# t-neumann/versalignLib

Hardware: AMD Instinct MI355X
Metric: GCUPS (giga DP cell updates/sec) SW affine-gap, 150x500 bp (higher is better)
Workload: dtype int16; 1 GPU; 1048576 pairs/GPU, 150 bp x 500 bp, SW affine-gap int16 score (open -5, extend -1), inputs resident in HBM; pairs_per_gpu=1048576, read_length=150, ref_length=500, kernel_geometry=8x19

## Files before the change

versalignlib_amd/csrc/cell_constants.h:

```cpp
#pragma once

namespace valign {

struct Scoring {
    int match = 2, mismatch = -1, gap_read = -3, gap_ref = -3;
    bool affine = false;
    int open_read = -3, ext_read = -3, open_ref = -3, ext_ref = -3;
};

constexpr int kAlgSW = 0;
constexpr int kAlgNW = 1;

constexpr int kGapLinear = 0, kGapSym = 1, kGapAffine = 2, kGapAffineSym = 3;
constexpr int kGapAffineSymF16 = 4, kGapAffineF16 = 5, kGapSymF16 = 6;
constexpr int kTiltMaxK = 12;
constexpr int kSideTileG = 8, kSideTileK = 19;
constexpr bool tilt_tables_only(int G, int K) { return G == kSideTileG && K == kSideTileK; }
constexpr bool tilt_frame_built(int G, int K) { return K <= kTiltMaxK || tilt_tables_only(G, K); }
constexpr int kSideTilePad = kSideTileG + 4, kSideTilePairs = 2 * (64 / kSideTileG);
constexpr int side_tile_refs_area(int F) { return ((kSideTilePairs * F + 32 + 15) / 16) * 16; }
constexpr int side_tile_stream_stride(int F) {
    const int dw = (F + 2 * kSideTilePad + 1) / 2;
    return 4 * (dw + ((kSideTileG - dw) % 64 + 64) % 64);
}
constexpr int side_tile_wave_lds(int R, int F) {
    const int streams = (64 / kSideTileG) * side_tile_stream_stride(F), raw_reads = ((kSideTilePairs * R + 32 + 15) / 16) * 16;
    return side_tile_refs_area(F) + (streams > raw_reads ? streams : raw_reads);
}

constexpr int kBandNwAbsent16 = -16384;
constexpr int kBandNwAbsent32 = -(1 << 29);

enum FillKernel {
    kFillLinear = 0,
    kFillLinearSym,
    kFillAffine,
    kFillSse,
    kFillTag,
    kFillTagKey,
    kFillAffineSym,
    kFillAffineTag,
    kFillAffineTagSym,
    kFillSseTag,
// ... 7 lines not shown
```

versalignlib_amd/csrc/cell_rules.h:

```cpp
#pragma once

#include <algorithm>
#include <cstdlib>
#include <stdexcept>
#include <string>

#include "cell_constants.h"
#include "extend_band_align_plan.h"

namespace valign {

struct RuleInputs {
    Scoring sc;
    int R = 0, F = 0;
    bool sse_policy = false;
    bool no_sym = false, no_tag = false, no_f16 = false, no_prof_key = false;
    bool no_max3 = false;
    bool no_tilt = false;
    bool no_row_tables = false;
    bool no_side_tile = false;
};

inline long long nw_tilt_span(const Scoring &sc, int rows, int F) {
    const long long per_row = -(long long)(sc.affine ? sc.ext_ref : sc.gap_ref);
    const long long per_col = -(long long)(sc.affine ? sc.ext_read : sc.gap_read);
    return per_row * (rows + 1) + per_col * (F + 1);
}

inline bool half_float_exact(const Scoring &sc, int alg, int R, int F, int rows) {
    const long long top = (long long)std::min(R, F) * std::max({sc.match, sc.mismatch, 0});
    long long slack = std::max({std::abs(sc.match), std::abs(sc.mismatch), std::abs(sc.open_read),
                                std::abs(sc.ext_read), std::abs(sc.open_ref), std::abs(sc.ext_ref)});
    if (alg == kAlgSW) return top + 2 * slack <= 2048 && slack <= 1024;
    if (!sc.affine) slack = std::max<long long>(slack, std::max(std::abs(sc.gap_read), std::abs(sc.gap_ref)));
    const long long span = nw_tilt_span(sc, rows, F);
// ... 123 lines not shown
    return std::max({sc.match, sc.mismatch, 0}) - 2 * sc.ext_ref + (sc.ext_ref - sc.open_ref);
}
inline bool sym_affine_row_tables_ok(const RuleInputs &in, int R, int F, int rows, int K, int lds_profile, int lds_tables) {
    if (in.no_row_tables || !sym_affine_tilt_ok(in, R, F, rows, K)) return false;
    if (in.sc.ext_ref - in.sc.open_ref < 0 || F > 60000) return false;
    return sym_affine_row_table_low(in.sc) >= 0 && sym_affine_row_table_high(in.sc) <= 255 && lds_tables <= lds_profile;
}
inline const char *ran_sym_affine_scores_name(bool row_tables) { return row_tables ? "row_tables" : "lds_profile"; }

constexpr int kSideTileRows = kSideTileG * kSideTileK, kSideTileMinRead = 129;
constexpr int kSideTileBlockWaves = 4, kSideTileLdsGranule = 2048, kSideTileLdsBudget = 152 * 1024;
inline bool side_tile_lds_ok(int lds_wave) {
    const long long block = ((long long)lds_wave * kSideTileBlockWaves + kSideTileLdsGranule - 1) / kSideTileLdsGranule * kSideTileLdsGranule;
    return lds_wave > 0 && 2 * block <= kSideTileLdsBudget;
}
inline const char *sym_affine_side_tile_refusal(const RuleInputs &in, int alg, int gaps, int R, int F, bool latency, bool forced) {
    const int lds_wave = side_tile_wave_lds(R, F);
    if (in.no_side_tile) return "the side tile is switched off (VALIGN_HIP_DEBUG=no_side_tile)";
    if (alg != kAlgSW) return "the 8 x 19 tile exists for Smith-Waterman scores only";
    if (gaps != kGapAffineSym)
        return "the 8 x 19 tile exists for int16 cells with symmetric affine gaps only (half_float_cells = 0, open_read = open_ref, ext_read = ext_ref)";
    if (R > kSideTileRows) return "the 8 x 19 tile holds reads of at most 152 bases";
    if (in.no_tilt) return "the 8 x 19 tile runs the tilted frame only (VALIGN_HIP_DEBUG=no_tilt)";
    if (in.no_row_tables) return "the 8 x 19 tile runs the row tables only (VALIGN_HIP_DEBUG=no_row_tables)";
    if (!sym_affine_row_tables_ok(in, in.R, in.F, kSideTileRows, kSideTileK, lds_wave, lds_wave))
        return "the 8 x 19 tile runs the tilted frame with row tables only: shape x scoring leave its window, or a substitution score of the frame is no byte (sym_affine_row_tables_ok)";
    if (!side_tile_lds_ok(lds_wave)) return "the 8 x 19 tile needs two 4-wave blocks per CU: the reference is too long for its LDS budget";
    if (forced) return "";
    if (R < kSideTileMinRead) return "reads of at most 128 bases fit a smaller tile";
    if (latency) return "small calls take the latency plan";
// ... 395 lines not shown
```

versalignlib_amd/csrc/dp_kernels.hip.h:

```cpp
#pragma once

#include <hip/hip_runtime.h>
#include <stdint.h>

#include <type_traits>
#include <utility>

#include "base_classes.h"
#include "cell_constants.h"
#include "lane_map.h"

namespace valign {

typedef short s16x2 __attribute__((ext_vector_type(2)));
typedef _Float16 f16x2 __attribute__((ext_vector_type(2)));
typedef unsigned short u16x2 __attribute__((ext_vector_type(2)));

constexpr int kWave = 64;
constexpr int kWaveLanes = 64;
constexpr int kCodePad = 72;
constexpr short kNegInf = -16384;

constexpr int kMaxScoreGroups = 16;
constexpr int kOneSweep = 0x7FFFFFFF;
// ... 396 lines not shown
    w.refc = refc + 2 * kCodePad;
    w.first_bad = first_bad;
    w.pair0 = pair0;
    w.last = last;
    return live;
}

constexpr int row_table_pad(int G) { return G + 4; }
constexpr unsigned kSelZero4 = 0x0c0c0c0cu;
constexpr unsigned kSelWiden = 0x04010400u;

template <int G, int K>
__device__ __forceinline__ bool wave_setup_tables(const uint8_t *reads, const uint8_t *refs, long long n, int R, int F,
                                                  int refs_area, int sel_stride, int wave_lds, short match, short mismatch,
                                                  short zero_score, short row0_score, unsigned block, WaveTables &w,
                                                  unsigned (&Ta)[K], unsigned (&Tb)[K], bool &repair) {
    using geo = Geo<G, K>;
    constexpr int kPad = row_table_pad(G);
    const int lane = threadIdx.x & (kWave - 1);
    const int wave = threadIdx.x / kWave;
    const int row0 = R - geo::kRows;

    unsigned char *raw = valign_smem + (size_t)wave * wave_lds;
    unsigned char *sel = raw + refs_area;

    const int waves = blockDim.x / kWave;
    const long long pair0 = ((long long)block * waves + wave) * geo::kPairs;
    const bool live = pair0 < n;
    long long pair_end = pair0 + geo::kPairs;
    if (pair_end > n) pair_end = n;
    const int last = (int)(pair_end - pair0) - 1;

    if (live) {
        stage_span(raw, refs, pair0 * F, pair_end * F, lane);
        stage_span(sel, reads, pair0 * R, pair_end * R, lane);
    }
    __syncthreads();

    if (live) {
        auto table = [&](int c, unsigned &lo, unsigned &hi) __attribute__((always_inline)) {
            unsigned b[8];
#pragma unroll
            for (int a = 0; a < 8; ++a) b[a] = (unsigned)(a >= 1 && a <= 4 ? (a == c + 1 ? match : mismatch) : zero_score) & 0xFFu;
            lo = b[0] | b[1] << 8 | b[2] << 16 | b[3] << 24;
            hi = b[4] | b[5] << 8 | b[6] << 16 | b[7] << 24;
        };
        unsigned t_lo[4], t_hi[4];
#pragma unroll
        for (int c = 0; c < 4; ++c) table(c, t_lo[c], t_hi[c]);
// ... 35 lines not shown
#pragma unroll
        for (int q = 0; q < K; ++q) {
            Ta[q] += r4;
            Tb[q] += r4;
        }
    }
    __syncthreads();

    int cols_used = 0;
    bool before_last = false;
    unsigned *stream = reinterpret_cast<unsigned *>(sel);
    const int stride_dw = sel_stride / 4;
    constexpr bool SEL16 = tilt_tables_only(G, K);
    unsigned short *stream16 = reinterpret_cast<unsigned short *>(sel);
    const int stride_h = sel_stride / 2;
    if (live) {
        for (int idx = lane; idx < geo::kGroups * 2 * kPad; idx += kWave) {
            const int g = idx / (2 * kPad), x = idx - g * (2 * kPad);
            if constexpr (SEL16) stream16[g * stride_h + (x < kPad ? x : F + x)] = (unsigned short)0x0c0c;
            else stream[g * stride_dw + (x < kPad ? x : F + x)] = kSelZero4;
        }
        const int ref_skew = (int)((unsigned long long)(refs + pair0 * F) & 15ull);
        typedef unsigned short u16;
#pragma unroll
        for (int g = 0; g < geo::kGroups; ++g) {
            int pa = 2 * g, pb = 2 * g + 1;
            pa = pa > last ? last : pa;
            pb = pb > last ? last : pb;
            const unsigned char *raw_a = raw + ref_skew + pa * F, *raw_b = raw + ref_skew + pb * F;
            unsigned *out_g = stream + g * stride_dw + kPad;
            unsigned short *out16_g = stream16 + g * stride_h + kPad;
            u16x2 ends_a = u16x2{0, 0}, ends_b = u16x2{0, 0};
            auto note = [](u16x2 &ends, unsigned acgt, int j) __attribute__((always_inline)) {
                const unsigned none = ~nonzero_bytes(acgt) & 0x80808080u;
                const u16 end = acgt ? (u16)(j + 4 - (__builtin_clz(acgt) >> 3)) : (u16)0;
                const u16 first_none = none ? (u16)(0xFFFF - (j + (__builtin_ctz(none) >> 3))) : (u16)0;
                ends = __builtin_elementwise_max(ends, u16x2{end, first_none});
            };
            const int F4 = F & ~3;
            for (int j = 4 * lane; j < F4; j += 4 * kWave) {
                const unsigned ca = base_class4(lds_dword_at(raw_a + j)), cb = base_class4(lds_dword_at(raw_b + j));
                const unsigned sa = select_bytes8(0x0c0c0c03u, 0x0201000cu, ca), sb = select_bytes8(0x0c0c0c07u, 0x0605040cu, cb);
                if constexpr (SEL16) {
                    uint2 s;
                    s.x = __builtin_amdgcn_perm(sb, sa, 0x05010400u);
                    s.y = __builtin_amdgcn_perm(sb, sa, 0x07030602u);
                    *reinterpret_cast<uint2 *>(out16_g + j) = s;
                } else {
                    uint4 s;
                    s.x = __builtin_amdgcn_perm(sb, sa, 0x0c040c00u) | 0x0c000c00u;
                    s.y = __builtin_amdgcn_perm(sb, sa, 0x0c050c01u) | 0x0c000c00u;
                    s.z = __builtin_amdgcn_perm(sb, sa, 0x0c060c02u) | 0x0c000c00u;
                    s.w = __builtin_amdgcn_perm(sb, sa, 0x0c070c03u) | 0x0c000c00u;
                    *reinterpret_cast<uint4 *>(out_g + j) = s;
                }
                note(ends_a, sa ^ kSelZero4, j);
                note(ends_b, sb ^ kSelZero4, j);
            }
            for (int j = F4 + lane; j < F; j += kWave) {
                const int ca = base_class(raw_a[j]), cb = base_class(raw_b[j]);
                const bool va = ca >= 1 && ca <= 4, vb = cb >= 1 && cb <= 4;
                if constexpr (SEL16) out16_g[j] = (unsigned short)((va ? (unsigned)(ca - 1) : 0x0cu) | (vb ? (unsigned)(cb + 3) : 0x0cu) << 8);
                else out_g[j] = (va ? (unsigned)(ca - 1) : 0x0cu) | (vb ? (unsigned)(cb + 3) : 0x0cu) << 16 | 0x0c000c00u;
                ends_a = __builtin_elementwise_max(ends_a, u16x2{va ? (u16)(j + 1) : (u16)0, va ? (u16)0 : (u16)(0xFFFF - j)});
                ends_b = __builtin_elementwise_max(ends_b, u16x2{vb ? (u16)(j + 1) : (u16)0, vb ? (u16)0 : (u16)(0xFFFF - j)});
            }
#pragma unroll
            for (int d = kWave / 2; d >= 1; d >>= 1) {
                ends_a = __builtin_elementwise_max(ends_a, __builtin_bit_cast(u16x2, __shfl_xor(__builtin_bit_cast(int, ends_a), d, kWave)));
                ends_b = __builtin_elementwise_max(ends_b, __builtin_bit_cast(u16x2, __shfl_xor(__builtin_bit_cast(int, ends_b), d, kWave)));
            }
            before_last |= 0xFFFF - (int)ends_a.y < (int)ends_a.x || 0xFFFF - (int)ends_b.y < (int)ends_b.x;
            cols_used = (int)ends_a.x > cols_used ? (int)ends_a.x : cols_used;
            cols_used = (int)ends_b.x > cols_used ? (int)ends_b.x : cols_used;
        }
    }
    __syncthreads();
    repair = __builtin_amdgcn_readfirstlane((int)before_last) != 0;
    w.cols_used = __builtin_amdgcn_readfirstlane(cols_used);
    w.prof = raw;
    w.refc = SEL16 ? reinterpret_cast<unsigned char *>(stream16 + kPad) : reinterpret_cast<unsigned char *>(stream + kPad);
    w.first_bad = nullptr;
    w.pair0 = pair0;
    w.last = last;
    return live;
}

template <int K>
__device__ __forceinline__ void lds_load_lane(unsigned addr, unsigned (&v)[K / 2]) {
// ... 32 lines not shown
    lds_load_lane<K>(addr_b, vb);
    merge_profile<K>(va, vb, S);
}



constexpr int kTrackAll = 0, kTrackNone = 1, kTrackPair = 2;

__host__ __device__ inline int nw_frame_centre(int R, int F, int rows, int match, int mismatch, int tilt_row, int tilt_col) {
    const int best = match > mismatch ? match : mismatch;
    const int top = (R < F ? R : F) * (best > 0 ? best : 0);
    return (top + tilt_row * (rows + 1) + tilt_col * (F + 1)) / 2;
}

template <int G, int K, int ALG, int GAPS>
__global__ void __launch_bounds__(256)
score_kernel(const ScoreArgs args) {
    using geo = Geo<G, K>;
    constexpr bool F16 = GAPS == kGapAffineSymF16 || GAPS == kGapAffineF16;
    constexpr bool F16SYM = GAPS == kGapAffineSymF16;
    constexpr bool AFFINE = GAPS == kGapAffine || GAPS == kGapAffineSym || F16;
    constexpr bool SYM = GAPS == kGapSym;
    constexpr bool LINF16 = GAPS == kGapSymF16;
    constexpr bool AFFSYM = GAPS == kGapAffineSym;
    constexpr bool SOURCES = AFFSYM && ALG == kAlgSW;
    const int lane = threadIdx.x & (kWave - 1);
    using lmap = LaneMap<G, score_lane_stride(G, K)>;
    static_assert(lmap::kInterleaved || (lmap::grp(kWave - 3) == (kWave - 3) / G && lmap::l(kWave - 3) == (kWave - 3) % G), "the contiguous map is lane / G, lane % G");
    const int grp = lmap::kInterleaved ? lmap::grp(lane) : lane / G;
    const int l = lmap::kInterleaved ? lmap::l(lane) : lane % G;

    const uint8_t *reads = args.reads, *refs = args.refs;
    int16_t *scores = args.scores;
    long long n_pairs = args.n;
    int F_batch = args.F;
    unsigned block = blockIdx.x;
    if (args.n_groups > 0) {
        int g = 0;
        while (g + 1 < args.n_groups && block >= args.groups[g].block_end) ++g;
        block -= g ? args.groups[g - 1].block_end : 0u;
        reads += args.groups[g].read_ofs;
        refs += args.groups[g].ref_ofs;
        scores += args.groups[g].pair_ofs;
        n_pairs = args.groups[g].n;
        F_batch = args.groups[g].F;
// ... 23 lines not shown
    auto cell_add = [](s16x2 a, s16x2 b) __attribute__((always_inline)) {
        return HALF ? __builtin_bit_cast(s16x2, __builtin_bit_cast(f16x2, a) + __builtin_bit_cast(f16x2, b)) : a + b;
    };
    auto cell_sub = [](s16x2 a, s16x2 b) __attribute__((always_inline)) {
        return HALF ? __builtin_bit_cast(s16x2, __builtin_bit_cast(f16x2, a) - __builtin_bit_cast(f16x2, b)) : a - b;
    };
    const short s_match = HALF ? __builtin_bit_cast(short, (_Float16)(((int)args.match + fold) * unit)) : (short)(args.match + fold);
    const short s_mismatch = HALF ? __builtin_bit_cast(short, (_Float16)(((int)args.mismatch + fold) * unit)) : (short)(args.mismatch + fold);
    const short s_zero = HALF ? __builtin_bit_cast(short, (_Float16)fold) : (short)fold;
    bool tables = false, repair = false;
    unsigned Ta[K], Tb[K];
    if constexpr (TABLES_ONLY) {
        tables = args.sym_max3_bias > 0 && (args.sym_max3_bias >> 16 & 3) == 3;
        if (!tables) return;
        if (!wave_setup_tables<G, K>(reads, refs, n_pairs, args.R, F_batch, args.prof_area, args.refc_stride, args.wave_lds,
                                     s_match, s_mismatch, s_zero, s_row0, block, w, Ta, Tb, repair))
            return;
        if (args.form_seen != nullptr && lane == 0) args.form_seen[repair ? 1 : 0] = 1u;
    } else if constexpr (TILT_BUILT) {
        tables = args.sym_max3_bias > 0 && (args.sym_max3_bias >> 16 & 3) == 3;
        bool live = false;
        if (tables)
            live = wave_setup_tables<G, K>(reads, refs, n_pairs, args.R, F_batch, args.prof_area, args.refc_stride, args.wave_lds,
                                           s_match, s_mismatch, s_zero, s_row0, block, w, Ta, Tb, repair);
        if (!tables)
            live = wave_setup<G, K, false>(reads, refs, n_pairs, args.R, F_batch, args.prof_area, args.refc_stride,
                                           args.wave_lds, s_match, s_mismatch, w, false, block, s_zero, kOneSweep, 0, s_row0);
        if (!live) return;
    } else if (!wave_setup<G, K, false>(reads, refs, n_pairs, args.R, F_batch, args.prof_area, args.refc_stride,
                                        args.wave_lds, s_match, s_mismatch, w, false, block, s_zero, kOneSweep, 0, s_row0))
        return;
// ... 506 lines not shown
            res = s16x2{(short)((int)b.x + rcentre), (short)((int)b.y + rcentre)};
        } else {
            res = s16x2{(short)(int)b.x, (short)(int)b.y};
        }
    } else if (ALG == kAlgSW) {
        res = best;
    } else {
        s16x2 col = l == G - 1 ? row_best : pk(0);
#pragma unroll
        for (int q = 0; q < K; ++q) col = pk_max(col, Hl[q] - cell(tilt_row * (l * K + q) + tilt_col * F));
        res = pk_max(col, pk(0));
    }
#pragma unroll
    for (int i = 0; i < lmap::kReduceSteps; ++i)
        res = pk_max(res, as_pk((unsigned)__shfl_xor((int)as_u32(res), lmap::reduce_distance(i), kWave)));
    if (l == 0) {
        const long long pa = pair0 + 2 * grp;
        if (pa + 1 < n_pairs && ((unsigned long long)scores & 3ull) == 0) {
            *reinterpret_cast<unsigned *>(scores + pa) = as_u32(res);
        } else {
            if (pa < n_pairs) scores[pa] = res.x;
            if (pa + 1 < n_pairs) scores[pa + 1] = res.y;
        }
    }
}

struct WaveLds {
    int prof_area, refc_stride, total;
};

template <int G, int K>
inline WaveLds wave_lds(int R, int F) {
// ... 33 lines not shown
```

versalignlib_amd/csrc/engine.hip.h:

```cpp
#pragma once

#include <hip/hip_runtime.h>
#include <stdint.h>
#include <stdio.h>
#include <stdlib.h>
#include <string.h>

#include <algorithm>
#include <atomic>
#include <chrono>
#include <condition_variable>
#include <functional>
#include <map>
#include <memory>
#include <mutex>
#include <stdexcept>
#include <string>
#include <thread>
#include <utility>
#include <vector>

#include "align_parts.h"
#include "cell_rules.h"
#include "hip_handles.h"
// ... 98 lines not shown
#undef VALIGN_COUNT

extern const Geometry kSideGeometry;

constexpr int kMaxBlockLds = 160 * 1024;
static_assert(kSideTileLdsBudget < kMaxBlockLds, "the side tile's LDS budget leaves a margin inside a CU's LDS");
constexpr int kSlots = 4;
constexpr int kDefaultBlockLds = 64 * 1024;

struct LaunchPlan {
    bool long_mode = false;
    const Geometry *geo = nullptr;
    WaveLds lds{};
    int waves_per_block = 4;
    int pairs_per_wave = 0;
};

class DebugSwitches {
public:
    DebugSwitches() {
        const char *env = getenv("VALIGN_HIP_DEBUG");
        if (!env) return;
        static const char *const known[] = {"no_sym", "no_tag", "no_f16", "no_max3", "no_tilt", "no_row_tables", "no_side_tile", "no_fused", "no_prof_key", "no_overlap", "no_band_chain",
                                            "force_long", "wide_align", "strip_k", "no_single_strip", "no_direct_out", "ragged_min", "chunk_bytes",
                                            "align_chunk_bytes", "direct_bytes", "scratch_cap_mb", "whole_rows", "short_strips", "cigar_rows_mb", "cigar_lanes",
                                            "span_scratch_bytes", "subopt_scratch_bytes", "span_cigar_mb"};
        std::string s(env);
        for (size_t at = 0; at <= s.size();) {
            const size_t end = std::min(s.find(',', at), s.size());
            const std::string item = s.substr(at, end - at);
            at = end + 1;
            if (item.empty()) continue;
            const size_t eq = item.find('=');
            const std::string name = item.substr(0, eq);
            bool ok = false;
            for (const char *k : known) ok = ok || name == k;
            if (!ok) throw std::runtime_error("VALIGN_HIP_DEBUG: unknown switch '" + name + "'");
            kv_[name] = eq == std::string::npos ? 1 : atoll(item.c_str() + eq + 1);
// ... 134 lines not shown
    void score_long_device(int alg, long long n, const uint8_t *d_reads, const uint8_t *d_refs, int16_t *d_scores, hipStream_t stream);
    void sync_band_tables(hipStream_t stream);
    void score_band_device(const LongScoreMode &mode, long long n, const uint8_t *d_reads, const uint8_t *d_refs, int16_t *d_scores, PlacedRec *d_placed,
                           hipStream_t stream);

    const char *score_cell_format(int alg, long long n = 0) const;
    std::string ran_score_cells() const;
    const char *ran_align_fill() const { return ran_align_fill_; }
    static std::string ran_geometry(const Geometry *g) { return g ? std::to_string(g->G) + "x" + std::to_string(g->K) : "none"; }
    std::string ran_kernels() const;

    RuleInputs rule_inputs() const {
        RuleInputs in = RuleInputs{sc_, R_, F_, sse_policy_, no_sym_, no_tag_, no_f16_, no_prof_key_, no_max3_, no_tilt_};
        in.no_row_tables = no_row_tables_;
        in.no_side_tile = no_side_tile_;
        return in;
    }
    bool score_int16_ok(int alg) const;
    bool score_wide_cells(int alg) const { return score_width_ == 32 || (score_width_ == 0 && !score_int16_ok(alg)); }

    void score_host(int opt, int n, const char *const *reads, const char *const *refs, short *scores,
                    int threads, int16_t *d_dest = nullptr);



    struct WalkChain {
        int region;
        long long chunk_pairs;
        int *min_start;
        uint8_t *packed;
// ... 138 lines not shown
    PlacedSweep extend_wide_sweep(ExtendRec *d_extend, bool banded = false) const;
    PlacedSweep extend_band_sweep() const;
    void score_placed_strips(const PlacedSweep &sweep, long long n, const uint8_t *d_reads, const uint8_t *d_refs, hipStream_t stream);
    static void raise_block_lds(const void *fn, int bytes) {
        if (bytes > kDefaultBlockLds)
            hip_check(hipFuncSetAttribute(fn, hipFuncAttributeMaxDynamicSharedMemorySize, bytes), "hipFuncSetAttribute(MaxDynamicSharedMemorySize)");
    }
    TraceArgs trace_args(int alg, const uint8_t *d_reads, const uint8_t *d_refs, long long n, const unsigned *ptr, const EndCell *ends, uint8_t *rows,
                         short *idx, int G, int K, int pad_rows, int blocks8) const;

    LaunchPlan choose_plan(int R, int F, int force_g, int force_k, bool latency = false, bool full_only = false) const;

    static LaunchPlan long_plan();

    LaunchPlan score_plan_for(const LaunchPlan &base, int alg, int R, int F, bool latency, bool refuse = true) const;
    static LaunchPlan side_plan(int R, int F);
    const char *side_tile_refusal(int alg, int R, int F, bool latency) const;
    bool few_pairs(long long n) const { return n > 0 && n <= (long long)latency_plan_.pairs_per_wave * 1024 && band_width_ == 0; }
    const char *ran_side_tile_form() const;
    void reset_side_tile_form(hipStream_t stream);


    long long whole_rounds(long long pairs, bool sw_scores = false) const;

    bool direct_call(long long n, size_t per_pair) const;

    void prime_copy_engines(hipStream_t copy_in, hipStream_t copy_out, long long staged_pairs);

    void flat_destination(FlatSink sink, long long n, uint8_t *&rows, short *&idx) const {
        if (HostRegistry::instance().covers(sink.rows, (size_t)n * 2 * sink.AL) &&
            HostRegistry::instance().covers(sink.idx, sizeof(short) * 4 * (size_t)n)) {
// ... 239 lines not shown
    std::vector<int> read_caps_, ref_caps_;
    std::vector<unsigned char> read_class_;
    std::vector<unsigned short> ref_class_;
    std::map<std::pair<int, int>, LaunchPlan> class_plans_;
    hipStream_t ragged_dev_stream_ = nullptr;
    HostPacker packer_{R_, F_};
    HostStats host_stats_;
    DebugSwitches dbg_;
    bool no_sym_ = dbg_.on("no_sym");
    bool no_tag_ = dbg_.on("no_tag");
    bool no_f16_ = dbg_.on("no_f16");
    bool no_max3_ = dbg_.on("no_max3");
    bool no_tilt_ = dbg_.on("no_tilt");
    bool no_row_tables_ = dbg_.on("no_row_tables");
    bool no_side_tile_ = dbg_.on("no_side_tile");
    bool side_forced_ = false;
    bool no_fused_ = dbg_.on("no_fused");
    bool no_prof_key_ = dbg_.on("no_prof_key");
    bool copy_engines_primed_ = false;
    std::unique_ptr<CopyIssuer> copy_issuer_;
    bool wide_align_ = dbg_.on("wide_align");
    bool whole_rows_ = dbg_.on("whole_rows");
    bool no_direct_out_ = dbg_.on("no_direct_out");
    bool no_overlap_ = dbg_.on("no_overlap");
    int strip_k_ = (int)dbg_.value("strip_k", 0);
    long long scratch_cap_mb_ = dbg_.value("scratch_cap_mb", 0);
    bool chain_regions_busy_[2] = {false, false};
    std::string arch_;
    LaunchPlan plan_, latency_plan_;
    LaunchPlan base_plan_;
// ... 3 lines not shown
    long long staged_pairs_ = 0, align_staged_pairs_ = 0;
    size_t record_staged_bytes_ = 0;
    bool pack_ = true;
    BandPlan band_plan_;
    int band_tables_width_ = -1;
    int band_blocks_per_cu_ = 0, band_lds_ = 0;
    int long_strip_rows_ = 0;
    static constexpr unsigned kRanF16 = 1, kRanInt16 = 2, kRanInt32 = 4;
    unsigned ran_score_cells_ = 0;
    const char *ran_align_fill_ = "none";
    const Geometry *ran_score_geo_ = nullptr, *ran_align_geo_ = nullptr;
    const Geometry *ran_placed_geo_ = nullptr, *ran_subopt_geo_ = nullptr, *ran_extend_geo_ = nullptr;
    const char *ran_score_sym_affine_ = nullptr;
    const char *ran_score_sym_affine_frame_ = "plain";
    const char *ran_score_sym_affine_scores_ = "lds_profile";
    const char *ran_placed_ = "none";
    std::string ran_span_ = "none";
    size_t span_scratch_bytes_ = (size_t)dbg_.value("span_scratch_bytes", 256ll << 20);
    std::string ran_span_cigar_ = "none";
    size_t span_cigar_bytes_ = (size_t)std::max(0ll, dbg_.value("span_cigar_mb", 768)) << 20;
    const char *ran_subopt_ = "none";
    int subopt_ring_cols_ = 0;
    size_t subopt_scratch_bytes_ = (size_t)dbg_.value("subopt_scratch_bytes", 256ll << 20);
    const char *ran_extend_ = "none";
    const char *ran_extend_align_ = "none";
    const Geometry *ran_extend_align_geo_ = nullptr;
    long long ran_extend_align_chunks_ = 0;
    const char *ran_result_format_ = "rows";
    int ran_cigar_lanes_ = 0;
    long long cigar_d2h_bytes_ = 0;
// ... 54 lines not shown
```

versalignlib_amd/csrc/engine_core.hip:

```cpp
#include <numeric>

#include "engine.hip.h"

namespace valign {

static WaveLds side_tile_lds(int R, int F) { return row_table_lds16(R, F); }
static Geometry side_geometry() {
    Geometry g{kSideTileG, kSideTileK, false, &side_tile_lds, {}, {}, [](int, int) -> const void * { return nullptr; },
               [](int, int) -> const void * { return nullptr; }, [](int) -> const void * { return nullptr; }, [](int) -> const void * { return nullptr; }};
    g.kernel[kAlgSW][kGapAffineSym] = (const void *)&score_kernel<kSideTileG, kSideTileK, kAlgSW, kGapAffineSym>;
    return g;
}
const Geometry kSideGeometry = side_geometry();

Engine::Engine(int device, int R, int F, const Scoring &sc, int force_g, int force_k)
    : device_(device), R_(R), F_(F), sc_(sc) {
    if (R < 0 || F < 0) throw std::runtime_error("negative sequence length");
    if ((long long)R + F > 32767)
        throw std::runtime_error("read_length + ref_length exceeds the ABI's 16-bit coordinates");
    validate_scoring();
    int count = 0;
    hip_check(hipGetDeviceCount(&count), "hipGetDeviceCount");
    if (device < 0 || device >= count)
        throw std::runtime_error("HIP device " + std::to_string(device) + " not present (" +
// ... 109 lines not shown
             (long long)(d_cig_rows_[0].bytes() + d_cig_rows_[1].bytes()), ran_placed_, placed_wide(), (long long)(d_placed_rows_.bytes() + d_placed_ends_.bytes()),
             ran_span_.c_str(), span_ref_length(rule_inputs()), (long long)span_[kSlots].bytes(),
             ran_span_cigar_.c_str(), (long long)(span_cigar_[0].bytes() + span_cigar_[1].bytes()),
             ran_subopt_, (long long)subopt_[kSlots].bytes(), subopt_ring_cols_, ran_extend_, extend_wide(), extend_band(), VALIGN_HIP_EXTEND_BAND_BLOCK_ROWS,
             ran_geometry(ran_score_geo_).c_str(), ran_geometry(ran_align_geo_).c_str(),
             ran_geometry(ran_placed_geo_).c_str(), ran_geometry(ran_subopt_geo_).c_str(), ran_geometry(ran_extend_geo_).c_str());
    std::string out(buf);
    out.insert(out.size() - 1, std::string(", \"ran_extend_align\": \"") + ran_extend_align_ + "\", \"ran_extend_align_geometry\": \"" +
                                   ran_geometry(ran_extend_align_geo_) + "\", \"extend_align_scratch_bytes\": " +
                                   std::to_string((long long)(d_ptr_.bytes() + d_ends_.bytes() + d_extend_align_recs_.bytes())) +
                                   ", \"extend_band_align\": " + std::to_string(extend_band_align()) + ", \"ran_extend_align_chunks\": " +
                                   std::to_string(ran_extend_align_chunks_) + ", \"ran_cigar_lanes\": " + std::to_string(ran_cigar_lanes_));
    if (ran_score_sym_affine_)
        out.insert(out.size() - 1, std::string(", \"ran_score_sym_affine\": \"") + ran_score_sym_affine_ + "\", \"ran_score_sym_affine_frame\": \"" +
                                       ran_score_sym_affine_frame_ + "\", \"ran_score_sym_affine_scores\": \"" + ran_score_sym_affine_scores_ + "\"");
    if (ran_score_sym_affine_ && ran_score_geo_ == &kSideGeometry)
        out.insert(out.size() - 1, std::string(", \"ran_score_sym_affine_form\": \"") + ran_side_tile_form() + "\"");
    return out;
}

void Engine::band_block_shape(int &block_rows, int &col_align) const {
    const bool chain = long_mode(kAlgSW, false).chain;
    block_rows = chain ? kBandK : VALIGN_HIP_BAND_BLOCK_ROWS;
    col_align = chain ? VALIGN_HIP_BAND_CHAIN_COL_ALIGN : VALIGN_HIP_BAND_COL_ALIGN;
}

void Engine::validate_scoring() {
    auto fits = [](int v) { return v >= -32768 && v <= 32767; };
    if (!fits(sc_.match) || !fits(sc_.mismatch) || !fits(sc_.gap_read) || !fits(sc_.gap_ref) ||
        !fits(sc_.open_read) || !fits(sc_.ext_read) || !fits(sc_.open_ref) || !fits(sc_.ext_ref))
        throw std::runtime_error("scoring parameter outside int16");
    const bool gaps_ok = sc_.affine ? (sc_.open_read <= 0 && sc_.ext_read <= 0 && sc_.open_ref <= 0 && sc_.ext_ref <= 0)
// ... 39 lines not shown
        if (latency) cost = (double)(F + g.G - 1) * (g.K * (sc_.affine ? 9.3 : 5.6) + 7.0);
        if (!best.geo || cost < best_cost) {
            best = p;
            best_cost = cost;
        }
    }
    if (!best.geo || (dbg_.on("force_long") && !force_g)) {
        if (force_g || force_k)
            throw std::runtime_error("the forced kernel geometry does not fit read_length=" + std::to_string(R) +
                                     ", ref_length=" + std::to_string(F));
        return long_plan();
    }
    return best;
}

LaunchPlan Engine::side_plan(int R, int F) {
    LaunchPlan p;
    p.geo = &kSideGeometry;
    p.lds = kSideGeometry.lds(R, F);
    p.waves_per_block = kSideTileBlockWaves;
    p.pairs_per_wave = 2 * (kWave / kSideTileG);
    return p;
}

const char *Engine::side_tile_refusal(int alg, int R, int F, bool latency) const {
    const RuleInputs in = rule_inputs();
    const int gaps = alg <= kAlgNW ? score_gap_form(in, alg, R, F, kSideTileRows) : -1;
    return sym_affine_side_tile_refusal(in, alg, gaps, R, F, latency, side_forced_);
}

const char *Engine::ran_side_tile_form() const {
    if (!d_form_seen_.get()) return "none";
    unsigned seen[2] = {0, 0};
    hip_check(hipSetDevice(device_), "hipSetDevice");
// ... 146 lines not shown
```

versalignlib_amd/csrc/engine_score.hip:

```cpp
#define VALIGN_TU_SCORE 1
#include "engine.hip.h"

namespace valign {

void Engine::score_device(int opt, long long n, const uint8_t *d_reads, const uint8_t *d_refs,
                  int16_t *d_scores, hipStream_t stream, bool length_sorted) {
    const int alg = opt & 0xF;
    if (alg > 1 || n <= 0) return;
    hip_check(hipSetDevice(device_), "hipSetDevice");
    if (length_sorted) {
        host_stats_ = HostStats{};
        ran_score_cells_ = 0;
        ran_score_geo_ = nullptr;
        ran_score_sym_affine_ = nullptr;
        reset_side_tile_form(stream);
    }
    if (score_width_ == 16 && !score_int16_ok(alg))
        throw std::runtime_error("shape x scoring can leave the int16 range of the DP cells (read_length " +
                                 std::to_string(R_) + ", ref_length " + std::to_string(F_) + ")");
    const bool wide = score_wide_cells(alg);
    if (side_forced_ && (plan_.long_mode || wide || band_width_ > 0))
        throw std::runtime_error("group_lanes = 8, rows_per_lane = 19: the call takes the long-read kernels (a band, int32 cells, or a reference too long for the register sweep)");
    if (plan_.long_mode || wide) {
        score_long_device(alg, n, d_reads, d_refs, d_scores, stream);
// ... 52 lines not shown
    ran_score_geo_ = plan.geo;
    if (alg == kAlgSW && gaps == kGapAffineSym) {
        const bool max3 = sym_affine_max3_ok(rule_inputs(), R_, F_);
        a.sym_max3_bias = max3 ? sym_affine_bias(sc_) : 0;
        const bool tilted = sym_affine_tilt_ok(rule_inputs(), R_, F_, plan.geo->G * plan.geo->K, plan.geo->K);
        if (tilted) a.sym_max3_bias = sym_affine_tilt_bias(sc_) | 1 << 16;
        const WaveLds tables_lds = tilt_tables_only(plan.geo->G, plan.geo->K) ? plan.lds : row_table_lds(plan.geo->G, R, F);
        const bool row_tables = tilted && sym_affine_row_tables_ok(rule_inputs(), R_, F_, plan.geo->G * plan.geo->K, plan.geo->K, plan.lds.total, tables_lds.total);
        if (tilt_tables_only(plan.geo->G, plan.geo->K)) {
            if (!row_tables) throw std::runtime_error("the 8 x 19 side tile was planned for a launch whose row tables are refused");
            if (!d_form_seen_.get()) {
                d_form_seen_.reserve(2 * sizeof(unsigned), "side tile form words");
                hip_check(hipMemset(d_form_seen_.get(), 0, 2 * sizeof(unsigned)), "hipMemset(form words)");
            }
            a.form_seen = d_form_seen_.get();
        }
        if (row_tables) {
            a.sym_max3_bias |= 1 << 17;
            a.prof_area = tables_lds.prof_area;
            a.refc_stride = tables_lds.refc_stride;
            a.wave_lds = tables_lds.total;
        }
        ran_score_sym_affine_ = ran_sym_affine_name(max3);
        ran_score_sym_affine_frame_ = ran_sym_affine_frame_name(tilted);
        ran_score_sym_affine_scores_ = ran_sym_affine_scores_name(row_tables);
    }
    const int block_lds = a.wave_lds * plan.waves_per_block;
    if (block_lds > kDefaultBlockLds)
        hip_check(hipFuncSetAttribute(fn, hipFuncAttributeMaxDynamicSharedMemorySize, block_lds),
                  "hipFuncSetAttribute(MaxDynamicSharedMemorySize)");
    if (blocks > 0x7FFFFFFFll) throw std::runtime_error("batch too large for one launch");
    if (blocks == 0) return;
    void *kargs[] = {&a};
    hip_check(hipLaunchKernel(fn, dim3((unsigned)blocks), dim3(plan.waves_per_block * kWave), kargs,
                              (size_t)block_lds, stream),
              "hipLaunchKernel(score_kernel)");
}

void Engine::launch_unpack(const uint8_t *d_packed, uint8_t *d_out, long long n, int len, hipStream_t stream) {
    if (n <= 0 || len <= 0) return;
    UnpackArgs a{d_packed, d_out, n, len};
    void *kargs[] = {&a};
// ... 358 lines not shown
```

Before: 10690 GCUPS.

## Stage side-tile references in halves to fit three blocks per CU

```diff
diff --git a/versalignlib_amd/csrc/cell_constants.h b/versalignlib_amd/csrc/cell_constants.h
--- a/versalignlib_amd/csrc/cell_constants.h
+++ b/versalignlib_amd/csrc/cell_constants.h
@@ -27,6 +27,10 @@
     const int streams = (64 / kSideTileG) * side_tile_stream_stride(F), raw_reads = ((kSideTilePairs * R + 32 + 15) / 16) * 16;
     return side_tile_refs_area(F) + (streams > raw_reads ? streams : raw_reads);
 }
+constexpr int side_tile_refs_half_area(int F) { return ((kSideTilePairs / 2 * F + 32 + 15) / 16) * 16; }
+constexpr int side_tile_half_staged_wave_lds(int R, int F) {
+    return side_tile_wave_lds(R, F) - side_tile_refs_area(F) + side_tile_refs_half_area(F);
+}
 
 constexpr int kBandNwAbsent16 = -16384;
 constexpr int kBandNwAbsent32 = -(1 << 29);
diff --git a/versalignlib_amd/csrc/cell_rules.h b/versalignlib_amd/csrc/cell_rules.h
--- a/versalignlib_amd/csrc/cell_rules.h
+++ b/versalignlib_amd/csrc/cell_rules.h
@@ -19,6 +19,7 @@
     bool no_tilt = false;
     bool no_row_tables = false;
     bool no_side_tile = false;
+    bool no_side_tile_3 = false;
 };
 
 inline long long nw_tilt_span(const Scoring &sc, int rows, int F) {
@@ -172,6 +173,25 @@
     const long long block = ((long long)lds_wave * kSideTileBlockWaves + kSideTileLdsGranule - 1) / kSideTileLdsGranule * kSideTileLdsGranule;
     return lds_wave > 0 && 2 * block <= kSideTileLdsBudget;
 }
+constexpr int kSideTileTwoBlockLds = 56 * 1024;
+inline bool side_tile_lds_ok3(int lds_wave) {
+    const long long block = ((long long)lds_wave * kSideTileBlockWaves + kSideTileLdsGranule - 1) / kSideTileLdsGranule * kSideTileLdsGranule;
+    return lds_wave > 0 && 3 * block <= kSideTileLdsBudget;
+}
+struct SideTileLayout {
+    int blocks_per_cu;
+    bool half_staged;
+    int refs_area;
+    int wave_lds;
+    int block_lds;
+};
+inline SideTileLayout side_tile_layout(const RuleInputs &in, int R, int F) {
+    const int half = side_tile_half_staged_wave_lds(R, F), full = side_tile_wave_lds(R, F);
+    if (!in.no_side_tile_3 && side_tile_lds_ok3(half))
+        return SideTileLayout{3, true, side_tile_refs_half_area(F), half, half * kSideTileBlockWaves};
+    return SideTileLayout{2, false, side_tile_refs_area(F), full, std::max(full * kSideTileBlockWaves, kSideTileTwoBlockLds)};
+}
+
 inline const char *sym_affine_side_tile_refusal(const RuleInputs &in, int alg, int gaps, int R, int F, bool latency, bool forced) {
     const int lds_wave = side_tile_wave_lds(R, F);
     if (in.no_side_tile) return "the side tile is switched off (VALIGN_HIP_DEBUG=no_side_tile)";
diff --git a/versalignlib_amd/csrc/dp_kernels.hip.h b/versalignlib_amd/csrc/dp_kernels.hip.h
--- a/versalignlib_amd/csrc/dp_kernels.hip.h
+++ b/versalignlib_amd/csrc/dp_kernels.hip.h
@@ -434,9 +434,10 @@
 __device__ __forceinline__ bool wave_setup_tables(const uint8_t *reads, const uint8_t *refs, long long n, int R, int F,
                                                   int refs_area, int sel_stride, int wave_lds, short match, short mismatch,
                                                   short zero_score, short row0_score, unsigned block, WaveTables &w,
-                                                  unsigned (&Ta)[K], unsigned (&Tb)[K], bool &repair) {
+                                                  unsigned (&Ta)[K], unsigned (&Tb)[K], bool &repair, bool half_staged = false) {
     using geo = Geo<G, K>;
     constexpr int kPad = row_table_pad(G);
+    constexpr int kHalfPairs = geo::kPairs / 2, kHalfGroups = geo::kGroups / 2;
     const int lane = threadIdx.x & (kWave - 1);
     const int wave = threadIdx.x / kWave;
     const int row0 = R - geo::kRows;
@@ -451,8 +452,9 @@
     if (pair_end > n) pair_end = n;
     const int last = (int)(pair_end - pair0) - 1;
 
+    const bool second_half = half_staged && last >= kHalfPairs;
     if (live) {
-        stage_span(raw, refs, pair0 * F, pair_end * F, lane);
+        stage_span(raw, refs, pair0 * F, (second_half ? pair0 + kHalfPairs : pair_end) * F, lane);
         stage_span(sel, reads, pair0 * R, pair_end * R, lane);
     }
     __syncthreads();
@@ -518,65 +520,147 @@
     constexpr bool SEL16 = tilt_tables_only(G, K);
     unsigned short *stream16 = reinterpret_cast<unsigned short *>(sel);
     const int stride_h = sel_stride / 2;
-    if (live) {
-        for (int idx = lane; idx < geo::kGroups * 2 * kPad; idx += kWave) {
-            const int g = idx / (2 * kPad), x = idx - g * (2 * kPad);
-            if constexpr (SEL16) stream16[g * stride_h + (x < kPad ? x : F + x)] = (unsigned short)0x0c0c;
-            else stream[g * stride_dw + (x < kPad ? x : F + x)] = kSelZero4;
-        }
-        const int ref_skew = (int)((unsigned long long)(refs + pair0 * F) & 15ull);
+    if constexpr (!SEL16) {
+        if (live) {
+            for (int idx = lane; idx < geo::kGroups * 2 * kPad; idx += kWave) {
+                const int g = idx / (2 * kPad), x = idx - g * (2 * kPad);
+                if constexpr (SEL16) stream16[g * stride_h + (x < kPad ? x : F + x)] = (unsigned short)0x0c0c;
+                else stream[g * stride_dw + (x < kPad ? x : F + x)] = kSelZero4;
+            }
+            const int ref_skew = (int)((unsigned long long)(refs + pair0 * F) & 15ull);
+            typedef unsigned short u16;
+#pragma unroll
+            for (int g = 0; g < geo::kGroups; ++g) {
+                int pa = 2 * g, pb = 2 * g + 1;
+                pa = pa > last ? last : pa;
+                pb = pb > last ? last : pb;
+                const unsigned char *raw_a = raw + ref_skew + pa * F, *raw_b = raw + ref_skew + pb * F;
+                unsigned *out_g = stream + g * stride_dw + kPad;
+                unsigned short *out16_g = stream16 + g * stride_h + kPad;
+                u16x2 ends_a = u16x2{0, 0}, ends_b = u16x2{0, 0};
+                auto note = [](u16x2 &ends, unsigned acgt, int j) __attribute__((always_inline)) {
+                    const unsigned none = ~nonzero_bytes(acgt) & 0x80808080u;
+                    const u16 end = acgt ? (u16)(j + 4 - (__builtin_clz(acgt) >> 3)) : (u16)0;
+                    const u16 first_none = none ? (u16)(0xFFFF - (j + (__builtin_ctz(none) >> 3))) : (u16)0;
+                    ends = __builtin_elementwise_max(ends, u16x2{end, first_none});
+                };
+                const int F4 = F & ~3;
+                for (int j = 4 * lane; j < F4; j += 4 * kWave) {
+                    const unsigned ca = base_class4(lds_dword_at(raw_a + j)), cb = base_class4(lds_dword_at(raw_b + j));
+                    const unsigned sa = select_bytes8(0x0c0c0c03u, 0x0201000cu, ca), sb = select_bytes8(0x0c0c0c07u, 0x0605040cu, cb);
+                    if constexpr (SEL16) {
+                        uint2 s;
+                        s.x = __builtin_amdgcn_perm(sb, sa, 0x05010400u);
+                        s.y = __builtin_amdgcn_perm(sb, sa, 0x07030602u);
+                        *reinterpret_cast<uint2 *>(out16_g + j) = s;
+                    } else {
+                        uint4 s;
+                        s.x = __builtin_amdgcn_perm(sb, sa, 0x0c040c00u) | 0x0c000c00u;
+                        s.y = __builtin_amdgcn_perm(sb, sa, 0x0c050c01u) | 0x0c000c00u;
+                        s.z = __builtin_amdgcn_perm(sb, sa, 0x0c060c02u) | 0x0c000c00u;
+                        s.w = __builtin_amdgcn_perm(sb, sa, 0x0c070c03u) | 0x0c000c00u;
+                        *reinterpret_cast<uint4 *>(out_g + j) = s;
+                    }
+                    note(ends_a, sa ^ kSelZero4, j);
+                    note(ends_b, sb ^ kSelZero4, j);
+                }
+                for (int j = F4 + lane; j < F; j += kWave) {
+                    const int ca = base_class(raw_a[j]), cb = base_class(raw_b[j]);
+                    const bool va = ca >= 1 && ca <= 4, vb = cb >= 1 && cb <= 4;
+                    if constexpr (SEL16) out16_g[j] = (unsigned short)((va ? (unsigned)(ca - 1) : 0x0cu) | (vb ? (unsigned)(cb + 3) : 0x0cu) << 8);
+                    else out_g[j] = (va ? (unsigned)(ca - 1) : 0x0cu) | (vb ? (unsigned)(cb + 3) : 0x0cu) << 16 | 0x0c000c00u;
+                    ends_a = __builtin_elementwise_max(ends_a, u16x2{va ? (u16)(j + 1) : (u16)0, va ? (u16)0 : (u16)(0xFFFF - j)});
+                    ends_b = __builtin_elementwise_max(ends_b, u16x2{vb ? (u16)(j + 1) : (u16)0, vb ? (u16)0 : (u16)(0xFFFF - j)});
+                }
+#pragma unroll
+                for (int d = kWave / 2; d >= 1; d >>= 1) {
+                    ends_a = __builtin_elementwise_max(ends_a, __builtin_bit_cast(u16x2, __shfl_xor(__builtin_bit_cast(int, ends_a), d, kWave)));
+                    ends_b = __builtin_elementwise_max(ends_b, __builtin_bit_cast(u16x2, __shfl_xor(__builtin_bit_cast(int, ends_b), d, kWave)));
+                }
+                before_last |= 0xFFFF - (int)ends_a.y < (int)ends_a.x || 0xFFFF - (int)ends_b.y < (int)ends_b.x;
+                cols_used = (int)ends_a.x > cols_used ? (int)ends_a.x : cols_used;
+                cols_used = (int)ends_b.x > cols_used ? (int)ends_b.x : cols_used;
+            }
+        }
+    } else {
         typedef unsigned short u16;
-#pragma unroll
-        for (int g = 0; g < geo::kGroups; ++g) {
-            int pa = 2 * g, pb = 2 * g + 1;
-            pa = pa > last ? last : pa;
-            pb = pb > last ? last : pb;
-            const unsigned char *raw_a = raw + ref_skew + pa * F, *raw_b = raw + ref_skew + pb * F;
-            unsigned *out_g = stream + g * stride_dw + kPad;
-            unsigned short *out16_g = stream16 + g * stride_h + kPad;
-            u16x2 ends_a = u16x2{0, 0}, ends_b = u16x2{0, 0};
-            auto note = [](u16x2 &ends, unsigned acgt, int j) __attribute__((always_inline)) {
-                const unsigned none = ~nonzero_bytes(acgt) & 0x80808080u;
-                const u16 end = acgt ? (u16)(j + 4 - (__builtin_clz(acgt) >> 3)) : (u16)0;
-                const u16 first_none = none ? (u16)(0xFFFF - (j + (__builtin_ctz(none) >> 3))) : (u16)0;
-                ends = __builtin_elementwise_max(ends, u16x2{end, first_none});
-            };
-            const int F4 = F & ~3;
-            for (int j = 4 * lane; j < F4; j += 4 * kWave) {
-                const unsigned ca = base_class4(lds_dword_at(raw_a + j)), cb = base_class4(lds_dword_at(raw_b + j));
-                const unsigned sa = select_bytes8(0x0c0c0c03u, 0x0201000cu, ca), sb = select_bytes8(0x0c0c0c07u, 0x0605040cu, cb);
-                if constexpr (SEL16) {
-                    uint2 s;
-                    s.x = __builtin_amdgcn_perm(sb, sa, 0x05010400u);
-                    s.y = __builtin_amdgcn_perm(sb, sa, 0x07030602u);
-                    *reinterpret_cast<uint2 *>(out16_g + j) = s;
-                } else {
-                    uint4 s;
-                    s.x = __builtin_amdgcn_perm(sb, sa, 0x0c040c00u) | 0x0c000c00u;
-                    s.y = __builtin_amdgcn_perm(sb, sa, 0x0c050c01u) | 0x0c000c00u;
-                    s.z = __builtin_amdgcn_perm(sb, sa, 0x0c060c02u) | 0x0c000c00u;
-                    s.w = __builtin_amdgcn_perm(sb, sa, 0x0c070c03u) | 0x0c000c00u;
-                    *reinterpret_cast<uint4 *>(out_g + j) = s;
-                }
-                note(ends_a, sa ^ kSelZero4, j);
-                note(ends_b, sb ^ kSelZero4, j);
-            }
-            for (int j = F4 + lane; j < F; j += kWave) {
-                const int ca = base_class(raw_a[j]), cb = base_class(raw_b[j]);
-                const bool va = ca >= 1 && ca <= 4, vb = cb >= 1 && cb <= 4;
-                if constexpr (SEL16) out16_g[j] = (unsigned short)((va ? (unsigned)(ca - 1) : 0x0cu) | (vb ? (unsigned)(cb + 3) : 0x0cu) << 8);
-                else out_g[j] = (va ? (unsigned)(ca - 1) : 0x0cu) | (vb ? (unsigned)(cb + 3) : 0x0cu) << 16 | 0x0c000c00u;
-                ends_a = __builtin_elementwise_max(ends_a, u16x2{va ? (u16)(j + 1) : (u16)0, va ? (u16)0 : (u16)(0xFFFF - j)});
-                ends_b = __builtin_elementwise_max(ends_b, u16x2{vb ? (u16)(j + 1) : (u16)0, vb ? (u16)0 : (u16)(0xFFFF - j)});
-            }
-#pragma unroll
-            for (int d = kWave / 2; d >= 1; d >>= 1) {
-                ends_a = __builtin_elementwise_max(ends_a, __builtin_bit_cast(u16x2, __shfl_xor(__builtin_bit_cast(int, ends_a), d, kWave)));
-                ends_b = __builtin_elementwise_max(ends_b, __builtin_bit_cast(u16x2, __shfl_xor(__builtin_bit_cast(int, ends_b), d, kWave)));
-            }
-            before_last |= 0xFFFF - (int)ends_a.y < (int)ends_a.x || 0xFFFF - (int)ends_b.y < (int)ends_b.x;
-            cols_used = (int)ends_a.x > cols_used ? (int)ends_a.x : cols_used;
-            cols_used = (int)ends_b.x > cols_used ? (int)ends_b.x : cols_used;
+        auto build_group = [&](int g, const unsigned char *staged, int first) __attribute__((always_inline)) {
+            {
+                int pa = 2 * g, pb = 2 * g + 1;
+                pa = pa > last ? last : pa;
+                pb = pb > last ? last : pb;
+                const unsigned char *raw_a = staged + (pa - first) * F, *raw_b = staged + (pb - first) * F;
+                unsigned *out_g = stream + g * stride_dw + kPad;
+                unsigned short *out16_g = stream16 + g * stride_h + kPad;
+                u16x2 ends_a = u16x2{0, 0}, ends_b = u16x2{0, 0};
+                auto note = [](u16x2 &ends, unsigned acgt, int j) __attribute__((always_inline)) {
+                    const unsigned none = ~nonzero_bytes(acgt) & 0x80808080u;
+                    const u16 end = acgt ? (u16)(j + 4 - (__builtin_clz(acgt) >> 3)) : (u16)0;
+                    const u16 first_none = none ? (u16)(0xFFFF - (j + (__builtin_ctz(none) >> 3))) : (u16)0;
+                    ends = __builtin_elementwise_max(ends, u16x2{end, first_none});
+                };
+                const int F4 = F & ~3;
+                for (int j = 4 * lane; j < F4; j += 4 * kWave) {
+                    const unsigned ca = base_class4(lds_dword_at(raw_a + j)), cb = base_class4(lds_dword_at(raw_b + j));
+                    const unsigned sa = select_bytes8(0x0c0c0c03u, 0x0201000cu, ca), sb = select_bytes8(0x0c0c0c07u, 0x0605040cu, cb);
+                    if constexpr (SEL16) {
+                        uint2 s;
+                        s.x = __builtin_amdgcn_perm(sb, sa, 0x05010400u);
+                        s.y = __builtin_amdgcn_perm(sb, sa, 0x07030602u);
+                        *reinterpret_cast<uint2 *>(out16_g + j) = s;
+                    } else {
+                        uint4 s;
+                        s.x = __builtin_amdgcn_perm(sb, sa, 0x0c040c00u) | 0x0c000c00u;
+                        s.y = __builtin_amdgcn_perm(sb, sa, 0x0c050c01u) | 0x0c000c00u;
+                        s.z = __builtin_amdgcn_perm(sb, sa, 0x0c060c02u) | 0x0c000c00u;
+                        s.w = __builtin_amdgcn_perm(sb, sa, 0x0c070c03u) | 0x0c000c00u;
+                        *reinterpret_cast<uint4 *>(out_g + j) = s;
+                    }
+                    note(ends_a, sa ^ kSelZero4, j);
+                    note(ends_b, sb ^ kSelZero4, j);
+                }
+                for (int j = F4 + lane; j < F; j += kWave) {
+                    const int ca = base_class(raw_a[j]), cb = base_class(raw_b[j]);
+                    const bool va = ca >= 1 && ca <= 4, vb = cb >= 1 && cb <= 4;
+                    if constexpr (SEL16) out16_g[j] = (unsigned short)((va ? (unsigned)(ca - 1) : 0x0cu) | (vb ? (unsigned)(cb + 3) : 0x0cu) << 8);
+                    else out_g[j] = (va ? (unsigned)(ca - 1) : 0x0cu) | (vb ? (unsigned)(cb + 3) : 0x0cu) << 16 | 0x0c000c00u;
+                    ends_a = __builtin_elementwise_max(ends_a, u16x2{va ? (u16)(j + 1) : (u16)0, va ? (u16)0 : (u16)(0xFFFF - j)});
+                    ends_b = __builtin_elementwise_max(ends_b, u16x2{vb ? (u16)(j + 1) : (u16)0, vb ? (u16)0 : (u16)(0xFFFF - j)});
+                }
+#pragma unroll
+                for (int d = kWave / 2; d >= 1; d >>= 1) {
+                    ends_a = __builtin_elementwise_max(ends_a, __builtin_bit_cast(u16x2, __shfl_xor(__builtin_bit_cast(int, ends_a), d, kWave)));
+                    ends_b = __builtin_elementwise_max(ends_b, __builtin_bit_cast(u16x2, __shfl_xor(__builtin_bit_cast(int, ends_b), d, kWave)));
+                }
+                before_last |= 0xFFFF - (int)ends_a.y < (int)ends_a.x || 0xFFFF - (int)ends_b.y < (int)ends_b.x;
+                cols_used = (int)ends_a.x > cols_used ? (int)ends_a.x : cols_used;
+                cols_used = (int)ends_b.x > cols_used ? (int)ends_b.x : cols_used;
+            }
+        };
+        if (live) {
+            for (int idx = lane; idx < geo::kGroups * 2 * kPad; idx += kWave) {
+                const int g = idx / (2 * kPad), x = idx - g * (2 * kPad);
+                if constexpr (SEL16) stream16[g * stride_h + (x < kPad ? x : F + x)] = (unsigned short)0x0c0c;
+                else stream[g * stride_dw + (x < kPad ? x : F + x)] = kSelZero4;
+            }
+            const int ref_skew = (int)((unsigned long long)(refs + pair0 * F) & 15ull);
+#pragma unroll
+            for (int g = 0; g < (SEL16 ? kHalfGroups : geo::kGroups); ++g) build_group(g, raw + ref_skew, 0);
+        }
+        if constexpr (SEL16) {
+            if (half_staged) {
+                __syncthreads();
+                if (live && second_half) stage_span(raw, refs, (pair0 + kHalfPairs) * F, pair_end * F, lane);
+                __syncthreads();
+            }
+            if (live) {
+                const int skew2 = (int)((unsigned long long)(refs + (pair0 + kHalfPairs) * F) & 15ull);
+                const int skew1 = (int)((unsigned long long)(refs + pair0 * F) & 15ull);
+                const unsigned char *staged = second_half ? raw + skew2 : raw + skew1;
+                const int first = second_half ? kHalfPairs : 0;
+#pragma unroll
+                for (int g = kHalfGroups; g < geo::kGroups; ++g) build_group(g, staged, first);
+            }
         }
     }
     __syncthreads();
@@ -639,7 +723,7 @@
 }
 
 template <int G, int K, int ALG, int GAPS>
-__global__ void __launch_bounds__(256)
+__global__ void __launch_bounds__(256, tilt_tables_only(G, K) ? 3 : 1)
 score_kernel(const ScoreArgs args) {
     using geo = Geo<G, K>;
     constexpr bool F16 = GAPS == kGapAffineSymF16 || GAPS == kGapAffineF16;
@@ -654,6 +738,7 @@
     static_assert(lmap::kInterleaved || (lmap::grp(kWave - 3) == (kWave - 3) / G && lmap::l(kWave - 3) == (kWave - 3) % G), "the contiguous map is lane / G, lane % G");
     const int grp = lmap::kInterleaved ? lmap::grp(lane) : lane / G;
     const int l = lmap::kInterleaved ? lmap::l(lane) : lane % G;
+    const int wave_s = (SOURCES && tilt_tables_only(G, K)) ? __builtin_amdgcn_readfirstlane((int)(threadIdx.x / kWave)) : 0;
 
     const uint8_t *reads = args.reads, *refs = args.refs;
     int16_t *scores = args.scores;
@@ -707,7 +792,7 @@
         tables = args.sym_max3_bias > 0 && (args.sym_max3_bias >> 16 & 3) == 3;
         if (!tables) return;
         if (!wave_setup_tables<G, K>(reads, refs, n_pairs, args.R, F_batch, args.prof_area, args.refc_stride, args.wave_lds,
-                                     s_match, s_mismatch, s_zero, s_row0, block, w, Ta, Tb, repair))
+                                     s_match, s_mismatch, s_zero, s_row0, block, w, Ta, Tb, repair, (args.sym_max3_bias >> 18 & 1) != 0))
             return;
         if (args.form_seen != nullptr && lane == 0) args.form_seen[repair ? 1 : 0] = 1u;
     } else if constexpr (TILT_BUILT) {
@@ -1244,8 +1329,16 @@
 #pragma unroll
     for (int i = 0; i < lmap::kReduceSteps; ++i)
         res = pk_max(res, as_pk((unsigned)__shfl_xor((int)as_u32(res), lmap::reduce_distance(i), kWave)));
-    if (l == 0) {
-        const long long pa = pair0 + 2 * grp;
+    long long out_pair0 = pair0;
+    int out_grp = grp, out_l = l;
+    if constexpr (TABLES_ONLY) {
+        const int lane_now = (int)__builtin_amdgcn_mbcnt_hi(~0u, __builtin_amdgcn_mbcnt_lo(~0u, 0u));
+        out_grp = lmap::grp(lane_now);
+        out_l = lmap::l(lane_now);
+        out_pair0 = ((long long)block * (int)(blockDim.x / kWave) + wave_s) * geo::kPairs;
+    }
+    if (out_l == 0) {
+        const long long pa = out_pair0 + 2 * out_grp;
         if (pa + 1 < n_pairs && ((unsigned long long)scores & 3ull) == 0) {
             *reinterpret_cast<unsigned *>(scores + pa) = as_u32(res);
         } else {
diff --git a/versalignlib_amd/csrc/engine.hip.h b/versalignlib_amd/csrc/engine.hip.h
--- a/versalignlib_amd/csrc/engine.hip.h
+++ b/versalignlib_amd/csrc/engine.hip.h
@@ -136,6 +136,7 @@
     WaveLds lds{};
     int waves_per_block = 4;
     int pairs_per_wave = 0;
+    SideTileLayout side{};
 };
 
 class DebugSwitches {
@@ -143,7 +144,7 @@
     DebugSwitches() {
         const char *env = getenv("VALIGN_HIP_DEBUG");
         if (!env) return;
-        static const char *const known[] = {"no_sym", "no_tag", "no_f16", "no_max3", "no_tilt", "no_row_tables", "no_side_tile", "no_fused", "no_prof_key", "no_overlap", "no_band_chain",
+        static const char *const known[] = {"no_sym", "no_tag", "no_f16", "no_max3", "no_tilt", "no_row_tables", "no_side_tile", "no_side_tile_3", "no_fused", "no_prof_key", "no_overlap", "no_band_chain",
                                             "force_long", "wide_align", "strip_k", "no_single_strip", "no_direct_out", "ragged_min", "chunk_bytes",
                                             "align_chunk_bytes", "direct_bytes", "scratch_cap_mb", "whole_rows", "short_strips", "cigar_rows_mb", "cigar_lanes",
                                             "span_scratch_bytes", "subopt_scratch_bytes", "span_cigar_mb"};
@@ -308,6 +309,7 @@
         RuleInputs in = RuleInputs{sc_, R_, F_, sse_policy_, no_sym_, no_tag_, no_f16_, no_prof_key_, no_max3_, no_tilt_};
         in.no_row_tables = no_row_tables_;
         in.no_side_tile = no_side_tile_;
+        in.no_side_tile_3 = no_side_tile_3_;
         return in;
     }
     bool score_int16_ok(int alg) const;
@@ -476,7 +478,7 @@
     static LaunchPlan long_plan();
 
     LaunchPlan score_plan_for(const LaunchPlan &base, int alg, int R, int F, bool latency, bool refuse = true) const;
-    static LaunchPlan side_plan(int R, int F);
+    LaunchPlan side_plan(int R, int F) const;
     const char *side_tile_refusal(int alg, int R, int F, bool latency) const;
     bool few_pairs(long long n) const { return n > 0 && n <= (long long)latency_plan_.pairs_per_wave * 1024 && band_width_ == 0; }
     const char *ran_side_tile_form() const;
@@ -746,6 +748,7 @@
     bool no_tilt_ = dbg_.on("no_tilt");
     bool no_row_tables_ = dbg_.on("no_row_tables");
     bool no_side_tile_ = dbg_.on("no_side_tile");
+    bool no_side_tile_3_ = dbg_.on("no_side_tile_3");
     bool side_forced_ = false;
     bool no_fused_ = dbg_.on("no_fused");
     bool no_prof_key_ = dbg_.on("no_prof_key");
@@ -779,6 +782,8 @@
     const char *ran_score_sym_affine_ = nullptr;
     const char *ran_score_sym_affine_frame_ = "plain";
     const char *ran_score_sym_affine_scores_ = "lds_profile";
+    int ran_side_blocks_ = 0, ran_side_block_lds_ = 0;
+    bool ran_side_half_staged_ = false;
     const char *ran_placed_ = "none";
     std::string ran_span_ = "none";
     size_t span_scratch_bytes_ = (size_t)dbg_.value("span_scratch_bytes", 256ll << 20);
diff --git a/versalignlib_amd/csrc/engine_core.hip b/versalignlib_amd/csrc/engine_core.hip
--- a/versalignlib_amd/csrc/engine_core.hip
+++ b/versalignlib_amd/csrc/engine_core.hip
@@ -147,8 +147,16 @@
     if (ran_score_sym_affine_)
         out.insert(out.size() - 1, std::string(", \"ran_score_sym_affine\": \"") + ran_score_sym_affine_ + "\", \"ran_score_sym_affine_frame\": \"" +
                                        ran_score_sym_affine_frame_ + "\", \"ran_score_sym_affine_scores\": \"" + ran_score_sym_affine_scores_ + "\"");
-    if (ran_score_sym_affine_ && ran_score_geo_ == &kSideGeometry)
+    if (ran_score_sym_affine_ && ran_score_geo_ == &kSideGeometry) {
         out.insert(out.size() - 1, std::string(", \"ran_score_sym_affine_form\": \"") + ran_side_tile_form() + "\"");
+        int granted = 0;
+        hip_check(hipSetDevice(device_), "hipSetDevice");
+        hip_check(hipOccupancyMaxActiveBlocksPerMultiprocessor(&granted, kSideGeometry.kernel[kAlgSW][kGapAffineSym], kSideTileBlockWaves * kWave,
+                                                               (size_t)ran_side_block_lds_),
+                  "hipOccupancyMaxActiveBlocksPerMultiprocessor(score_kernel<8, 19>)");
+        out.insert(out.size() - 1, ", \"side_tile_blocks_planned\": " + std::to_string(ran_side_blocks_) + ", \"side_tile_blocks_granted\": " + std::to_string(granted) +
+                                       ", \"side_tile_layout\": \"" + (ran_side_half_staged_ ? "half_staged" : "single_pass") + "\"");
+    }
     return out;
 }
 
@@ -218,10 +226,13 @@
     return best;
 }
 
-LaunchPlan Engine::side_plan(int R, int F) {
+LaunchPlan Engine::side_plan(int R, int F) const {
     LaunchPlan p;
     p.geo = &kSideGeometry;
+    p.side = side_tile_layout(rule_inputs(), R, F);
     p.lds = kSideGeometry.lds(R, F);
+    p.lds.prof_area = p.side.refs_area;
+    p.lds.total = p.side.wave_lds;
     p.waves_per_block = kSideTileBlockWaves;
     p.pairs_per_wave = 2 * (kWave / kSideTileG);
     return p;
diff --git a/versalignlib_amd/csrc/engine_score.hip b/versalignlib_amd/csrc/engine_score.hip
--- a/versalignlib_amd/csrc/engine_score.hip
+++ b/versalignlib_amd/csrc/engine_score.hip
@@ -90,6 +90,7 @@
                 hip_check(hipMemset(d_form_seen_.get(), 0, 2 * sizeof(unsigned)), "hipMemset(form words)");
             }
             a.form_seen = d_form_seen_.get();
+            if (plan.side.half_staged) a.sym_max3_bias |= 1 << 18;
         }
         if (row_tables) {
             a.sym_max3_bias |= 1 << 17;
@@ -101,7 +102,13 @@
         ran_score_sym_affine_frame_ = ran_sym_affine_frame_name(tilted);
         ran_score_sym_affine_scores_ = ran_sym_affine_scores_name(row_tables);
     }
-    const int block_lds = a.wave_lds * plan.waves_per_block;
+    int block_lds = a.wave_lds * plan.waves_per_block;
+    if (plan.side.blocks_per_cu) {
+        block_lds = plan.side.block_lds;
+        ran_side_blocks_ = plan.side.blocks_per_cu;
+        ran_side_block_lds_ = block_lds;
+        ran_side_half_staged_ = plan.side.half_staged;
+    }
     if (block_lds > kDefaultBlockLds)
         hip_check(hipFuncSetAttribute(fn, hipFuncAttributeMaxDynamicSharedMemorySize, block_lds),
                   "hipFuncSetAttribute(MaxDynamicSharedMemorySize)");
```

Result: no change. 10800 GCUPS (median of 6 runs) (+1.0%).
